# atomicarchitects/equiformer

Hardware: AMD Instinct MI355X
Metric: molecules/sec (train step) QM9 L_max=2, 6 blocks (higher is better)
Workload: dtype f32; 1 GPU; QM9 graph_attention_transformer_nonlinear_l2 train step (radius graph + fwd + L1 + bwd + AdamW), 128 molecules/GPU x 18 atoms, r=5.0, num_basis=128, alpha_drop=0.2; global_batch=128, nodes_per_gpu=2304, edges_per_gpu=25354, parallelism=dp1, matrix_mode=split, hip_graph=True, hip_graph_replays=449, hip_graph_eager_steps=3

## Files before the change

### equiformer_amd/csrc/edge.hip

```cpp
#include "common.h"
#include "prof.h"

namespace {

__global__ __launch_bounds__(256) void gather_add_kernel(const float* __restrict__ a, const float* __restrict__ b,
                                                         const int* __restrict__ src, const int* __restrict__ dst,
                                                         float* __restrict__ msg, long total4, int D4) {
  const long idx = (long)blockIdx.x * blockDim.x + threadIdx.x;
  if (idx >= total4) return;
  const long e = idx / D4;
  const int c = (int)(idx - e * D4);
  float4 v = reinterpret_cast<const float4*>(a)[(long)src[e] * D4 + c];
  if (b) {
    const float4 w = reinterpret_cast<const float4*>(b)[(long)dst[e] * D4 + c];
    v.x += w.x, v.y += w.y, v.z += w.z, v.w += w.w;
  }
  reinterpret_cast<float4*>(msg)[idx] = v;
}

__global__ __launch_bounds__(128) void segment_sum_kernel(const float* __restrict__ x, const int* __restrict__ ptr,
                                                          const int* __restrict__ perm, float* __restrict__ out, int D,
                                                          float scale, int accumulate) {
  const int n = blockIdx.x;
  const int beg = ptr[n], end = ptr[n + 1];
  if ((D & 3) == 0) {
    const int D4 = D >> 2;
    for (int c = threadIdx.x; c < D4; c += blockDim.x) {
      float4 acc = make_float4(0.f, 0.f, 0.f, 0.f);
      for (int q = beg; q < end; q += 4) {
        long row[4];
        float4 v[4];
#pragma unroll
        for (int j = 0; j < 4; ++j) {
          const int qq = min(q + j, end - 1);
          row[j] = perm ? perm[qq] : qq;
        }
#pragma unroll
        for (int j = 0; j < 4; ++j) v[j] = reinterpret_cast<const float4*>(x)[row[j] * D4 + c];
#pragma unroll
        for (int j = 0; j < 4; ++j)
          if (q + j < end) acc.x += v[j].x, acc.y += v[j].y, acc.z += v[j].z, acc.w += v[j].w;
      }
      acc.x *= scale, acc.y *= scale, acc.z *= scale, acc.w *= scale;
      float4* o = reinterpret_cast<float4*>(out) + (long)n * D4 + c;
      if (accumulate) {
        const float4 p = *o;
        acc.x += p.x, acc.y += p.y, acc.z += p.z, acc.w += p.w;
      }
      *o = acc;
    }
  } else {
    for (int c = threadIdx.x; c < D; c += blockDim.x) {
      float acc = 0.f;
      for (int q = beg; q < end; ++q) {
        const long row = perm ? perm[q] : q;
        acc += x[row * D + c];
      }
      acc *= scale;
      float* o = out + (long)n * D + c;
      *o = accumulate ? *o + acc : acc;
    }
  }
}

__global__ __launch_bounds__(256) void segment_bcast_kernel(const float* __restrict__ x, const int* __restrict__ seg_of,
                                                            float* __restrict__ out, long total, int D, float scale) {
  const long idx = (long)blockIdx.x * blockDim.x + threadIdx.x;
  if (idx >= total) return;
  const long row = idx / D;
  const int c = (int)(idx - row * D);
  out[idx] = scale * x[(long)seg_of[row] * D + c];
}

__global__ __launch_bounds__(256) void segment_scale_kernel(const float* __restrict__ x, const float* __restrict__ s,
                                                            const int* __restrict__ seg_of, float* __restrict__ out,
                                                            long total4, int D4) {
  const long idx = (long)blockIdx.x * blockDim.x + threadIdx.x;
  if (idx >= total4) return;
  const long row = idx / D4;
  const float f = s[seg_of[row]];
  float4 v = reinterpret_cast<const float4*>(x)[idx];
  v.x *= f; v.y *= f; v.z *= f; v.w *= f;
  reinterpret_cast<float4*>(out)[idx] = v;
}

// ... 454 lines not shown

int eqf_gather_add_fwd(const float* a, const float* b, const int* src, const int* dst, float* msg, int E, int D,
                       void* stream) {
  if (!a || !src || !msg || (b && !dst)) return EQF_E_BADARG;
  if (D % 4 != 0) return EQF_E_UNSUPPORTED;
  if (E <= 0) return 0;
  const long total4 = (long)E * (D / 4);
  hipLaunchKernelGGL(gather_add_kernel, dim3(eqf_cdiv(total4, 256)), dim3(256), 0, (hipStream_t)stream, a, b, src, dst,
                     msg, total4, D / 4);
  EQF_CHECK_LAUNCH();
  return 0;
}

int eqf_segment_sum(const float* x, const int* ptr, const int* perm, float* out, int nseg, int D, float scale,
                    int accumulate, void* stream) {
  if (!x || !ptr || !out) return EQF_E_BADARG;
  if (nseg <= 0 || D <= 0) return 0;
  hipLaunchKernelGGL(segment_sum_kernel, dim3(nseg), dim3(128), 0, (hipStream_t)stream, x, ptr, perm, out, D, scale,
                     accumulate);
  EQF_CHECK_LAUNCH();
  return 0;
}

int eqf_segment_scale(const float* x, const float* s, const int* seg_of, float* out, int rows, int D, void* stream) {
  if (!x || !s || !seg_of || !out) return EQF_E_BADARG;
  if (D % 4) return EQF_E_UNSUPPORTED;
  if (rows <= 0 || D <= 0) return 0;
  const long total4 = (long)rows * (D / 4);
  hipLaunchKernelGGL(segment_scale_kernel, dim3(eqf_cdiv(total4, 256)), dim3(256), 0, (hipStream_t)stream, x, s, seg_of,
                     out, total4, D / 4);
  EQF_CHECK_LAUNCH();
  return 0;
}

int eqf_segment_bcast(const float* x, const int* seg_of, float* out, int rows, int D, float scale, void* stream) {
  if (!x || !seg_of || !out) return EQF_E_BADARG;
  if (rows <= 0 || D <= 0) return 0;
  const long total = (long)rows * D;
  hipLaunchKernelGGL(segment_bcast_kernel, dim3(eqf_cdiv(total, 256)), dim3(256), 0, (hipStream_t)stream, x, seg_of,
                     out, total, D, scale);
  EQF_CHECK_LAUNCH();
  return 0;
}

int eqf_dtp_coupling_fwd(const float* sh, const float* cg, const eqf_dtp_paths* paths, float* coupling, int E,
                         void* stream) {
// ... 148 lines not shown
```

### equiformer_amd/csrc/rowops.hip

```cpp
#include "common.h"

namespace {

constexpr int WAVES_PER_BLOCK = 4;

struct SegTab {
  int nseg;
  int off[EQF_MAX_SEG];
  int len[EQF_MAX_SEG];
  int mul[EQF_MAX_SEG];
  int l[EQF_MAX_SEG];
  int woff[EQF_MAX_SEG];
  int boff[EQF_MAX_SEG];
  int zidx[EQF_MAX_SEG];
  int n0;
  int D;
};

SegTab make_segtab(const eqf_irreps& ir) {
  SegTab t{};
  t.nseg = ir.nseg;
  int off = 0, w = 0, b = 0, n0 = 0;
  for (int s = 0; s < ir.nseg; ++s) {
    t.off[s] = off;
// ... 79 lines not shown
      for (int i = lane; i < n; i += 64) sum += xs[i];
      mean = wave_sum(sum) / n;
    }
    float sg = 0.f, sgx = 0.f;
    for (int i = lane; i < n; i += 64) {
      const float g = gs[i] * ws[i % mul];
      const float xh = (xs[i] - mean) * rs;
      sg += g;
      sgx += g * xh;
    }
    sgx = wave_sum(sgx) / n;
    sg = (T.l[s] == 0) ? wave_sum(sg) / n : 0.f;
    for (int i = lane; i < n; i += 64) {
      const float g = gs[i] * ws[i % mul];
      const float xh = (xs[i] - mean) * rs;
      float v = rs * (g - sg - xh * sgx);
      if (rr) v += rr[T.off[s] + i];
      dr[T.off[s] + i] = v;
    }
  }
}

constexpr int LN_WGRAD_ROWS = 64, LN_WGRAD_CHUNK = 16;
__global__ __launch_bounds__(256) void layernorm_wgrad_kernel(const float* __restrict__ x, const float* __restrict__ dy,
                                                              const float* __restrict__ rstd,
                                                              const float* __restrict__ mean0, float* __restrict__ dw,
                                                              float* __restrict__ db, int rows, SegTab T) {
  constexpr int CH = LN_WGRAD_CHUNK;
  const int c = blockIdx.x * blockDim.x + threadIdx.x;
  if (c >= T.D) return;
  int s = 0;
  while (s + 1 < T.nseg && c >= T.off[s + 1]) ++s;
  const int u = (c - T.off[s]) % T.mul[s];
  const bool is0 = T.l[s] == 0;
  const int n0 = T.n0, z = T.zidx[s];
  float aw = 0.f, ab = 0.f;
  for (int r0 = blockIdx.y * LN_WGRAD_ROWS; r0 < min(rows, (int)(blockIdx.y + 1) * LN_WGRAD_ROWS); r0 += CH) {
    float gv[CH], xs[CH], rs[CH], m0[CH];
#pragma unroll
    for (int k = 0; k < CH; ++k) {
      const int r = min(r0 + k, rows - 1);
      gv[k] = dy[(long)r * T.D + c];
      xs[k] = x[(long)r * T.D + c];
      rs[k] = rstd[(long)r * T.nseg + s];
      m0[k] = is0 ? mean0[(long)r * n0 + z] : 0.f;
    }
#pragma unroll
    for (int k = 0; k < CH; ++k) {
      const float g = (r0 + k < rows) ? gv[k] : 0.f;
      aw += g * (xs[k] - m0[k]) * rs[k];
      ab += g;
    }
  }
  atomicAdd(dw + T.woff[s] + u, aw);
  if (T.boff[s] >= 0) atomicAdd(db + T.boff[s] + u, ab);
}

struct GateTab {
  int S, G, nseg;
  int in_off[EQF_MAX_SEG], out_off[EQF_MAX_SEG], goff[EQF_MAX_SEG], mul[EQF_MAX_SEG], d[EQF_MAX_SEG];
  int Din, Dout;
};

GateTab make_gatetab(int S, const eqf_irreps& gated) {
  GateTab t{};
  t.S = S;
  t.nseg = gated.nseg;
  int G = 0;
  for (int s = 0; s < gated.nseg; ++s) G += gated.mul[s];
  t.G = G;
  int in_off = S + G, out_off = S, g = 0;
  for (int s = 0; s < gated.nseg; ++s) {
    t.in_off[s] = in_off, t.out_off[s] = out_off, t.goff[s] = S + g;
    t.mul[s] = gated.mul[s], t.d[s] = 2 * gated.l[s] + 1;
    in_off += t.mul[s] * t.d[s], out_off += t.mul[s] * t.d[s], g += t.mul[s];
  }
  t.Din = in_off, t.Dout = out_off;
  return t;
// ... 443 lines not shown
int eqf_layernorm_fwd(const float* x, const float* weight, const float* bias, float* y, float* rstd, float* mean0,
                      int rows, const eqf_irreps* irreps, float eps, void* stream) {
  return eqf_add_layernorm_fwd(x, nullptr, nullptr, weight, bias, y, rstd, mean0, rows, irreps, eps, stream);
}

int eqf_add_layernorm_bwd(const float* x, const float* weight, const float* dy, const float* dres, const float* rstd,
                          const float* mean0, float* dx, float* d_weight, float* d_bias, int rows,
                          const eqf_irreps* irreps, void* stream) {
  if (!x || !weight || !dy || !rstd || !mean0 || !dx || !irreps || irreps->nseg < 1 || irreps->nseg > EQF_MAX_SEG)
    return EQF_E_BADARG;
  if (rows <= 0) return 0;
  const SegTab T = make_segtab(*irreps);
  hipLaunchKernelGGL(layernorm_bwd_kernel, dim3(eqf_cdiv(rows, WAVES_PER_BLOCK)), dim3(256), 0, (hipStream_t)stream, x,
                     weight, dy, dres, rstd, dx, rows, T);
  EQF_CHECK_LAUNCH();
  if (d_weight && d_bias) {
    hipLaunchKernelGGL(layernorm_wgrad_kernel, dim3(eqf_cdiv(T.D, 256), eqf_cdiv(rows, LN_WGRAD_ROWS)), dim3(256), 0,
                       (hipStream_t)stream, x, dy, rstd, mean0, d_weight, d_bias, rows, T);
    EQF_CHECK_LAUNCH();
  }
  return 0;
}

int eqf_layernorm_bwd(const float* x, const float* weight, const float* dy, const float* rstd, const float* mean0,
                      float* dx, float* d_weight, float* d_bias, int rows, const eqf_irreps* irreps, void* stream) {
  return eqf_add_layernorm_bwd(x, weight, dy, nullptr, rstd, mean0, dx, d_weight, d_bias, rows, irreps, stream);
}

int eqf_gate_fwd(const float* in, float* out, int rows, int S, const eqf_irreps* gated, float c_silu, float c_sig,
                 void* stream) {
  if (!in || !out || !gated) return EQF_E_BADARG;
  if (rows <= 0) return 0;
  const GateTab T = make_gatetab(S, *gated);
  const int RB = 8;
  hipLaunchKernelGGL(gate_fwd_cols_kernel, dim3(eqf_cdiv(rows, RB), eqf_cdiv(T.Dout, 256)), dim3(256), 0,
                     (hipStream_t)stream, in, out, rows, T, c_silu, c_sig, RB);
  EQF_CHECK_LAUNCH();
  return 0;
}

int eqf_gate_bwd(const float* in, const float* d_out, float* d_in, int rows, int S, const eqf_irreps* gated,
                 float c_silu, float c_sig, void* stream) {
  if (!in || !d_out || !d_in || !gated) return EQF_E_BADARG;
  for (int s = 0; s < gated->nseg; ++s)
    if (gated->l[s] > 3) return EQF_E_UNSUPPORTED;
  if (rows <= 0) return 0;
// ... 124 lines not shown
```

### equiformer_amd/lib.py

```python
import ctypes
import os

_HERE = os.path.dirname(os.path.abspath(__file__))
LIB_PATH = os.path.join(_HERE, "libequiformer_hip.so")
if os.environ.get("EQF_LIB_VARIANT"):
    LIB_PATH = os.path.join(_HERE, "libequiformer_hip_%s.so" % os.environ["EQF_LIB_VARIANT"])

EQF_MAX_SEG = 8
EQF_MAX_PATHS = 72
EQF_L3_ODD = 0x100

c_fp = ctypes.c_void_p
c_int = ctypes.c_int


class EqfIrreps(ctypes.Structure):
    _fields_ = [("nseg", c_int), ("l", c_int * EQF_MAX_SEG), ("mul", c_int * EQF_MAX_SEG), ("odd", c_int * EQF_MAX_SEG)]


class EqfRows(ctypes.Structure):
    _fields_ = [("d", c_int), ("ld", c_int), ("inner", c_int)]


class EqfGemmDesc(ctypes.Structure):
    _fields_ = [("A", c_fp), ("B", c_fp), ("C", c_fp), ("bias", c_fp), ("ra", EqfRows), ("rc", EqfRows),
                ("ldb", c_int), ("M", c_int), ("N", c_int), ("K", c_int), ("accumulate", c_int), ("kind", c_int)]


class EqfGateIn(ctypes.Structure):
    _fields_ = [("S", c_int), ("G", c_int), ("c_silu", ctypes.c_float), ("c_sig", ctypes.c_float)]


_PA = c_int * EQF_MAX_PATHS


class EqfDtpPaths(ctypes.Structure):
    _fields_ = [("npaths", c_int), ("sh_dim", c_int), ("in_dim", c_int), ("out_dim", c_int), ("w_numel", c_int),
                ("m_numel", c_int), ("l1", _PA), ("l2", _PA), ("l3", _PA), ("mul", _PA), ("in_off", _PA),
                ("out_off", _PA), ("out_ch", _PA), ("out_k", _PA), ("w_off", _PA), ("cg_off", _PA), ("m_off", _PA)]


_SA = c_int * EQF_MAX_SEG


class EqfEdgeDeg(ctypes.Structure):
    _fields_ = [("nblk", c_int), ("C", c_int), ("H", c_int), ("w_numel", c_int), ("pw_numel", c_int), ("m_numel", c_int),
                ("Z", c_int), ("D", c_int), ("l", _SA), ("N", _SA), ("K", _SA), ("w_off", _SA), ("out_ch", _SA),
                ("pw_off", _SA), ("m_off", _SA), ("node_off", _SA), ("z_off", _SA)]

# ... 38 lines not shown
    "eqf_dtp_coupling_fwd": [c_fp, c_fp, _P_PATHS, c_fp, c_int, c_fp],
    "eqf_dtp_coupling_bwd": [c_fp, c_fp, _P_PATHS, c_fp, c_int, c_fp],
    "eqf_dtp_linear_fwd": [c_fp, c_fp, c_fp, _P_PATHS, _PP, c_fp, c_fp, _P_IRR, c_int, c_fp],
    "eqf_dtp_linear_wgrad": [c_fp, c_fp, c_fp, _P_PATHS, c_fp, _P_IRR, _PP, c_int, c_fp],
    "eqf_sfc_fwd": [c_fp, c_fp, c_fp, _P_PATHS, _PP, c_fp, c_fp, c_fp, c_fp, _P_IRR, c_fp, c_int, c_int, c_fp],
    "eqf_sfc_bwd_data": [c_fp, c_fp, c_fp, _P_PATHS, _PP, c_fp, c_fp, _P_IRR, c_fp, c_int, c_fp, c_fp, c_fp, c_int, c_fp],
    "eqf_sfc_bwd_weight": [c_fp, c_fp, c_fp, _P_PATHS, c_fp, _P_IRR, c_fp, c_int, _PP, c_fp, c_int, c_fp],
    "eqf_sfcx_packed_numel": [_P_PATHS, _P_IRR, c_int, c_int],
    "eqf_sfcx_supported": [_P_PATHS, _P_IRR, c_int, c_int],
    "eqf_sfcx_fwd_gated": [c_fp, ctypes.POINTER(EqfGateIn), c_fp, c_fp, _P_PATHS, c_fp, c_fp, c_fp, _P_IRR, c_int, c_int, c_fp],
    "eqf_sfcx_bwd_data_gated": [c_fp, ctypes.POINTER(EqfGateIn), c_fp, c_fp, _P_PATHS, c_fp, c_fp, _P_IRR, c_fp, c_fp, c_fp,
                                c_int, c_int, c_fp],
    "eqf_sfcx_bwd_weight_gated": [c_fp, ctypes.POINTER(EqfGateIn), c_fp, c_fp, _P_PATHS, c_fp, _P_IRR, _PP, c_int, c_int,
                                  c_fp],
    "eqf_sfcx_bwd_weight_bias": [c_fp, c_fp, c_fp, _P_PATHS, c_fp, _P_IRR, c_fp, c_int, _PP, c_fp, c_fp, c_fp, c_int, c_int, c_fp],
    "eqf_sfcx_bwd_weight_gated_bias": [c_fp, ctypes.POINTER(EqfGateIn), c_fp, c_fp, _P_PATHS, c_fp, _P_IRR, _PP, c_fp, c_int,
                                       c_int, c_fp],
    "eqf_sfcx_pack": [_PP, c_fp, _P_PATHS, _P_IRR, c_int, c_int, c_fp, c_fp],
    "eqf_sfcx_fwd": [c_fp, c_fp, c_fp, _P_PATHS, c_fp, c_fp, c_fp, c_fp, _P_IRR, c_fp, c_int, c_int, c_int, c_fp],
    "eqf_sfcx_bwd_data": [c_fp, c_fp, c_fp, _P_PATHS, c_fp, c_fp, _P_IRR, c_fp, c_int, c_fp, c_fp, c_fp, c_int, c_int, c_fp],
    "eqf_sfcx_bwd_weight": [c_fp, c_fp, c_fp, _P_PATHS, c_fp, _P_IRR, c_fp, c_int, _PP, c_fp, c_int, c_int, c_fp],
    "eqf_layernorm_fwd": [c_fp, c_fp, c_fp, c_fp, c_fp, c_fp, c_int, _P_IRR, _f, c_fp],
    "eqf_layernorm_bwd": [c_fp, c_fp, c_fp, c_fp, c_fp, c_fp, c_fp, c_fp, c_int, _P_IRR, c_fp],
    "eqf_add_layernorm_fwd": [c_fp, c_fp, c_fp, c_fp, c_fp, c_fp, c_fp, c_fp, c_int, _P_IRR, _f, c_fp],
    "eqf_add_layernorm_bwd": [c_fp, c_fp, c_fp, c_fp, c_fp, c_fp, c_fp, c_fp, c_fp, c_int, _P_IRR, c_fp],
    "eqf_graphnorm_fwd": [c_fp, c_fp, c_fp, c_fp, c_fp, c_fp, c_fp, c_fp, c_fp, c_fp, c_fp, c_int, c_int, _P_IRR, _f, c_fp],
    "eqf_graphnorm_bwd": [c_fp, c_fp, c_fp, c_fp, c_fp, c_fp, c_fp, c_fp, c_fp, c_fp, c_fp, c_fp, c_fp, c_fp, c_int, c_int,
                          _P_IRR, c_fp],
    "eqf_gate_fwd": [c_fp, c_fp, c_int, c_int, _P_IRR, _f, _f, c_fp],
    "eqf_gate_bwd": [c_fp, c_fp, c_fp, c_int, c_int, _P_IRR, _f, _f, c_fp],
    "eqf_silu_fwd": [c_fp, c_fp, _long, _f, c_fp],
    "eqf_silu_bwd": [c_fp, c_fp, c_fp, _long, _f, c_fp],
    "eqf_lnsilu_fwd": [c_fp, c_fp, c_fp, c_fp, c_int, c_int, _f, c_fp],
    "eqf_lnsilu_bwd": [c_fp, c_fp, c_fp, c_fp, c_fp, c_fp, c_fp, c_int, c_int, _f, c_fp],
    "eqf_lnsilu_group_fwd": [c_fp, c_fp, c_fp, c_fp, c_int, c_int, c_int, _f, c_fp],
    "eqf_lnsilu_group_bwd": [c_fp, c_fp, c_fp, c_fp, c_fp, c_fp, c_fp, c_int, c_int, c_int, _f, c_fp],
    "eqf_fold_weight_fwd": [c_fp, c_fp, c_fp, c_fp, c_fp, c_int, c_fp],
    "eqf_fold_weight_bwd": [c_fp, c_fp, c_fp, c_fp, c_fp, c_fp, c_fp, c_int, c_fp],
    "eqf_embed_fwd": [c_fp, c_fp, c_fp, c_fp, c_int, c_int, c_int, c_fp],
    "eqf_embed_bwd": [c_fp, c_fp, c_fp, c_fp, c_int, c_int, c_int, c_fp],
    "eqf_gather_add_fwd": [c_fp, c_fp, c_fp, c_fp, c_fp, c_int, c_int, c_fp],
    "eqf_segment_sum": [c_fp, c_fp, c_fp, c_fp, c_int, c_int, _f, c_int, c_fp],
    "eqf_segment_bcast": [c_fp, c_fp, c_fp, c_int, c_int, _f, c_fp],
    "eqf_kv_split": [c_fp, c_fp, c_fp, c_int, c_int, c_fp, c_fp],
    "eqf_kv_merge": [c_fp, c_fp, c_fp, c_int, c_int, c_fp, c_fp],
    "eqf_dp_logits_fwd": [c_fp, c_fp, c_fp, c_fp, c_int, c_int, c_fp, c_fp],
    "eqf_dp_logits_bwd": [c_fp, c_fp, c_fp, c_fp, c_fp, c_fp, c_int, c_int, c_fp, c_fp],
    "eqf_vec_sh": [c_fp, c_fp, c_int, c_int, _f, c_fp, c_fp],
    "eqf_edgedeg_fold_fwd": [c_fp, c_fp, c_fp, c_fp, c_fp, _P_EDEG, c_fp, c_fp, c_fp],
    "eqf_edgedeg_fold_bwd": [c_fp, c_fp, c_fp, c_fp, c_fp, _P_EDEG, c_fp, c_fp, c_fp, c_fp, c_fp, c_fp, c_fp],
    "eqf_edgedeg_scatter_fwd": [c_fp, c_fp, c_fp, c_fp, _P_EDEG, _f, c_fp, c_int, c_int, c_fp],
    "eqf_edgedeg_scatter_bwd": [c_fp, c_fp, c_fp, c_fp, _P_EDEG, _f, c_fp, c_fp, c_int, c_int, c_fp],
    "eqf_segment_scale": [c_fp, c_fp, c_fp, c_fp, c_int, c_int, c_fp],
    "eqf_dtp_fwd": [c_fp, c_fp, c_fp, _P_PATHS, c_fp, c_int, c_fp],
    "eqf_dtp_bwd": [c_fp, c_fp, c_fp, _P_PATHS, c_fp, c_fp, c_fp, c_fp, c_int, c_fp],
    "eqf_alpha_fwd": [c_fp, c_fp, c_fp, c_int, c_int, c_int, _f, c_fp],
    "eqf_alpha_bwd": [c_fp, c_fp, c_fp, c_fp, c_fp, c_int, c_int, c_int, _f, c_fp],
    "eqf_attn_aggregate_fwd": [c_fp, c_fp, c_fp, c_fp, c_fp, c_int, c_int, _P_IRR, _f, _u64, c_fp],
    "eqf_attn_aggregate_bwd": [c_fp, c_fp, c_fp, c_fp, c_fp, c_fp, c_int, c_int, _P_IRR, _f, _u64, c_fp],
    "eqf_attn_aggregate_fwd_dseed": [c_fp, c_fp, c_fp, c_fp, c_fp, c_int, c_int, _P_IRR, _f, _u64, c_fp, c_fp],
    "eqf_attn_aggregate_bwd_dseed": [c_fp, c_fp, c_fp, c_fp, c_fp, c_fp, c_int, c_int, _P_IRR, _f, _u64, c_fp, c_fp],
    "eqf_silu_bwd2": [c_fp, c_fp, c_fp, c_fp, c_fp, _long, _f, c_fp],
    "eqf_gate_bwd2": [c_fp, c_fp, c_fp, c_fp, c_fp, c_int, c_int, _P_IRR, _f, _f, c_fp],
    "eqf_lnsilu_bwd2": [c_fp, c_fp, c_fp, c_fp, c_fp, c_fp, c_fp, c_fp, c_fp, c_int, c_int, _f, c_fp],
    "eqf_lnsilu_group_bwd2": [c_fp, c_fp, c_fp, c_fp, c_fp, c_fp, c_fp, c_fp, c_fp, c_int, c_int, c_int, _f, c_fp],
# ... 111 lines not shown
```

### equiformer_amd/ops.py

```python
import contextlib
import ctypes
import os
import weakref

import torch
from torch.autograd import Function
from torch.autograd.function import once_differentiable

from . import lib
from .lib import EqfGemmDesc, EqfRows, call


class HipOnlyError(RuntimeError):
    pass


_dummy = {}


class _Flag:
    on = False


_input_grads_only = _Flag()


class input_grads_only:

    def __enter__(self):
        self.prev = _input_grads_only.on
        _input_grads_only.on = True

    def __exit__(self, *exc):
# ... 163 lines not shown
        n = x.shape[0]
        y = torch.empty_like(x)
        rstd = torch.empty((n, len(layout.segs)), device=x.device, dtype=torch.float32)
        mean0 = torch.empty((n, _ln_means(layout)), device=x.device, dtype=torch.float32)
        call("eqf_layernorm_fwd", _p(x), _p(weight), _p(bias), _p(y), _p(rstd), _p(mean0), n, layout.c_ref,
             float(eps), _stream())
        ctx.save_for_backward(x, weight, rstd, mean0, bias)
        ctx.layout = layout
        ctx.nb = bias.numel()
        ctx.eps = eps
        return y

    @staticmethod
    def backward(ctx, dy):
        x, weight, rstd, mean0, bias = ctx.saved_tensors
        if torch.is_grad_enabled():
            dx, dw, db = _LayerNormBwd.apply(x, weight, dy, rstd, mean0, ctx.layout, ctx.eps, ctx.nb)
            return dx, _guard(dw, dy, "layer-norm weight gradient"), _guard(db, dy, "layer-norm bias gradient"), \
                None, None
        dy = _c(dy)
        _chk(dy)
        dx = torch.empty_like(x)
        dw, db = _zeros2(weight.numel(), ctx.nb, x.device)
        call("eqf_layernorm_bwd", _p(x), _p(weight), _p(dy), _p(rstd), _p(mean0), _p(dx), _p(dw), _p(db), x.shape[0],
             ctx.layout.c_ref, _stream())
        return dx, dw, db, None, None


class _LayerNormBwd(Function):

    @staticmethod
    def forward(ctx, x, weight, dy, rstd, mean0, layout, eps, nb):
        dy = _c(dy)
        _chk(dy)
        dx = torch.empty_like(x)
        want = _want_param_grads()
        dw, db = _zeros2(weight.numel(), nb, x.device) if want else (None, None)
        call("eqf_layernorm_bwd", _p(x), _p(weight), _p(dy), _p(rstd), _p(mean0), _p(dx), _p(dw), _p(db), x.shape[0],
             layout.c_ref, _stream())
        ctx.save_for_backward(x, weight, dy)
        ctx.layout, ctx.eps = layout, eps
        if not want:
            return dx, None, None
        ctx.mark_non_differentiable(dw, db)
        return dx, dw, db

    @staticmethod
    @once_differentiable
# ... 5 lines not shown
        g_w = _zeros_like(weight)
        call("eqf_layernorm_bwd2", _p(x), _p(weight), _p(dy), _p(c), _p(g_x), _p(g_w), _p(g_dy), x.shape[0],
             ctx.layout.c_ref, float(ctx.eps), _stream())
        return g_x, g_w, g_dy, None, None, None, None, None


def layer_norm(x, weight, bias, layout, eps=1e-5):
    return _LayerNorm.apply(x, weight, bias, layout, eps)


class _AddLayerNorm(Function):

    @staticmethod
    def forward(ctx, a, b, weight, bias, layout, eps):
        a, b = _c(a), _c(b)
        _chk(a, b, weight, bias)
        n = a.shape[0]
        s = torch.empty_like(a)
        y = torch.empty_like(a)
        rstd = torch.empty((n, len(layout.segs)), device=a.device, dtype=torch.float32)
        mean0 = torch.empty((n, _ln_means(layout)), device=a.device, dtype=torch.float32)
        call("eqf_add_layernorm_fwd", _p(a), _p(b), _p(s), _p(weight), _p(bias), _p(y), _p(rstd), _p(mean0), n,
             layout.c_ref, float(eps), _stream())
        ctx.save_for_backward(s, weight, rstd, mean0)
        ctx.layout, ctx.nb, ctx.eps = layout, bias.numel(), eps
        return s, y

    @staticmethod
    def backward(ctx, ds, dy):
        s, weight, rstd, mean0 = ctx.saved_tensors
        if dy is None:
            return ds, ds, None, None, None, None
        if torch.is_grad_enabled():
            dx, dw, db = _LayerNormBwd.apply(s, weight, dy, rstd, mean0, ctx.layout, ctx.eps, ctx.nb)
            d = dx if ds is None else dx + ds
            return d, d, _guard(dw, dy, "layer-norm weight gradient"), _guard(db, dy, "layer-norm bias gradient"), \
                None, None
        dy = _c(dy)
        ds = _c(ds) if ds is not None else None
        _chk(dy, ds)
        d = torch.empty_like(s)
        want = _want_param_grads()
        dw, db = _zeros2(weight.numel(), ctx.nb, s.device) if want else (None, None)
        call("eqf_add_layernorm_bwd", _p(s), _p(weight), _p(dy), _p(ds), _p(rstd), _p(mean0), _p(d), _p(dw), _p(db), s.shape[0],
             ctx.layout.c_ref, _stream())
        return d, d, dw, db, None, None


def add_layer_norm(a, b, weight, bias, layout, eps=1e-5):
    return _AddLayerNorm.apply(a, b, weight, bias, layout, eps)


def _gn_graph(graph, n):
    if graph is None or getattr(graph, "batch", None) is None or getattr(graph, "mol_ptr", None) is None:
        raise ValueError("the graph / instance norm needs the batch's EdgeGraph (graph=...) with batch and mol_ptr")
    if graph.batch.shape[0] != n or graph.num_graphs <= 0:
        raise ValueError("graph norm: %d rows, but the graph has %d nodes in %d graphs"
                         % (n, graph.batch.shape[0], graph.num_graphs))
    _chk(graph.mol_ptr, graph.batch)
    return graph.mol_ptr, graph.batch, int(graph.num_graphs)


def _gn_fwd(a, b, mean_shift, weight, bias, layout, graph, eps):
    _chk(a, b, mean_shift, weight, bias)
    n = a.shape[0]
    mol_ptr, batch, B = _gn_graph(graph, n)
    s = torch.empty_like(a) if b is not None else None
    y = torch.empty_like(a)
# ... 166 lines not shown
                           n * d, K, N))
    return dx, descs


def _lin_dgrad(dy, weight, spec):
    dx, descs = _lin_dgrad_descs(dy, weight, spec)
    _gemm_group(descs, _stream())
    return dx


def _lin_wgrad_descs(x, dy, spec, dw, db=None):
    n = x.shape[0]
    Din, Dout = spec.in_layout.dim, spec.out_layout.dim
    descs = []
    for (l, in_off, K, out_off, N, w_off) in spec.pairs:
        d = 2 * l + 1
        descs.append(_desc(2, (x, in_off), rows(d, Din, K), (dy, out_off), N, (dw, w_off), rows(d, Dout, N),
                           db if spec.has_bias(l, out_off) else None, K, N, n * d))
    return descs



_defer_wgrad = [os.environ.get("EQF_DEFER_WGRAD", "1") != "0"]
_defer_stats = {"queued": 0, "flushes": 0}


class _TaskQueue:
    __slots__ = ("entries", "__weakref__")

    def __init__(self):
        self.entries = []


_task_queues = weakref.WeakValueDictionary()


def set_deferred_weight_gradients(on):
    prev = _defer_wgrad[0]
    _defer_wgrad[0] = bool(on)
    return prev


def deferred_weight_gradient_stats(reset=False):
    out = dict(_defer_stats)
    if reset:
        _defer_stats["queued"] = _defer_stats["flushes"] = 0
    return out


def _alias(t):
    return (t.untyped_storage(), t.storage_offset(), t.numel(), t.device)


def _from_alias(a):
    stor, off, n, dev = a
    return torch.empty(0, dtype=torch.float32, device=dev).set_(stor, off, (n,))


def _launch_queue(q, early=False):
    entries, q.entries = q.entries, []
    if early:
        ready = [e for e in entries if e[0].grad is not None and (not e[5] or e[1].grad is not None)]
        q.entries = [e for e in entries if not (e[0].grad is not None and (not e[5] or e[1].grad is not None))]
        entries = ready
    descs = []
    for (w, b, x, dy, spec, fused_b, aw, ab) in entries:
        tw = _from_alias(aw)
        if w.grad is not None and w.grad.data_ptr() != tw.data_ptr():
            tw = w.grad.view(-1)
        tb = None
        if fused_b:
            tb = _from_alias(ab)
            if b.grad is not None and b.grad.data_ptr() != tb.data_ptr():
                tb = b.grad.view(-1)
        if not tw.is_contiguous() or tw.dtype != torch.float32 or (tb is not None and not tb.is_contiguous()):
            raise RuntimeError("deferred weight gradient: .grad must be a contiguous fp32 tensor")
        descs += _lin_wgrad_descs(x, dy, spec, tw, tb)
    if descs:
        _defer_stats["flushes"] += 1
        _gemm_group(descs, _stream())


def flush_deferred_weight_gradients():
    try:
        task = torch._C._current_graph_task_id()
    except Exception:
        return
    q = _task_queues.get(task)
    if q is not None and q.entries:
        _launch_queue(q, early=True)


def _hooked(p):
    if getattr(p, "_eqf_flushes", False):
        return False
    if getattr(p, "_backward_hooks", None) or getattr(p, "_post_accumulate_grad_hooks", None):
        return True
    dist = torch.distributed
    return bool(dist.is_available() and dist.is_initialized())


def _accumulates_into_grad(p):
    try:
        return bool(torch._C._will_engine_execute_node(torch.autograd.graph.get_gradient_edge(p).node))
    except RuntimeError:
        return False


def _can_defer(*params):
    return (_defer_wgrad[0] and not torch.is_grad_enabled()
            and all(p is None or (p.is_leaf and p.requires_grad and p.grad is None and not _hooked(p)
                                  and _accumulates_into_grad(p))
                    for p in params))


def _defer_lin_wgrad(w, b, x, dy, spec, fused_b, dw, db):
    task = torch._C._current_graph_task_id()
    q = _task_queues.get(task)
    if q is None:
        q = _TaskQueue()
        _task_queues[task] = q
        torch.autograd.Variable._execution_engine.queue_callback(lambda q=q: _launch_queue(q))
    q.entries.append((w, b, x, dy, spec, fused_b, _alias(dw), _alias(db) if fused_b else None))
    _defer_stats["queued"] += 1


def _launch(built):
    _gemm_group(built[1], _stream())
    return built[0]


def _lin_fwd(x, weight, bias, spec):
    return _launch(_lin_fwd_descs(x, weight, bias, spec))


def _lin_dgrad(dy, weight, spec):
    return _launch(_lin_dgrad_descs(dy, weight, spec))


def _lin_wgrad(x, dy, spec, dw, db=None):
    _gemm_group(_lin_wgrad_descs(x, dy, spec, dw, db), _stream())
    return dw


def _glin_fwd_descs(x, ldx, K, wide, Ws, bs, cols=None):
    G = len(Ws)
    cols = range(G) if cols is None else cols
# ... 718 lines not shown
        db = None
        if has_b and ctx.needs_input_grad[2] and _want_param_grads():
            db = torch.empty(spec.blocks[0]["N"], device=dnode.device, dtype=torch.float32)
        call("eqf_edgedeg_scatter_bwd", _p(dnode), _p(coupling), _p(graph.dst), _p(graph.row_ptr), spec.c_ref, scale, _p(dz),
             _p(db), graph.N, graph.E, _stream())
        return dz, None, db, None, None, None


def edgedeg_scatter(z, coupling, bias, graph, spec, scale):
    return _EdgeDegScatter.apply(z, coupling, bias, graph, spec, float(scale))


def _gather_add_fwd(a, b, graph):
    D = a.shape[1]
    msg = torch.empty((graph.E, D), device=a.device, dtype=torch.float32)
    call("eqf_gather_add_fwd", _p(a), _p(b), _p(graph.src), _p(graph.dst), _p(msg), graph.E, D, _stream())
    return msg


def _gather_add_bwd(dmsg, g, n, want_a, want_b):
    D = dmsg.shape[1]
    st = _stream()
    da = db = None
    if want_a:
        da = torch.empty((n, D), device=dmsg.device, dtype=torch.float32)
        call("eqf_segment_sum", _p(dmsg), _p(g.src_ptr), _p(g.src_perm), _p(da), n, D, 1.0, 0, st)
    if want_b:
        db = torch.empty((n, D), device=dmsg.device, dtype=torch.float32)
        call("eqf_segment_sum", _p(dmsg), _p(g.row_ptr), None, _p(db), n, D, 1.0, 0, st)
    return da, db


class _GatherAddBwd(Function):

    @staticmethod
    def forward(ctx, dmsg, graph, n, has_b):
        dmsg = _c(dmsg)
        _chk(dmsg)
        ctx.graph, ctx.has_b = graph, has_b
        da, db = _gather_add_bwd(dmsg, graph, n, True, has_b)
        if has_b:
            return da, db
        return da

    @staticmethod
    @once_differentiable
# ... 1384 lines not shown
```

### include/equiformer_hip.h

```cpp
#ifndef EQUIFORMER_HIP_H
#define EQUIFORMER_HIP_H

#ifdef __cplusplus
extern "C" {
#endif

#define EQF_MAX_SEG 8
#define EQF_MAX_PATHS 72

#define EQF_L3_ODD 0x100

#define EQF_E_BADARG (-1)
#define EQF_E_UNSUPPORTED (-2)

typedef struct eqf_irreps {
  int nseg;
  int l[EQF_MAX_SEG];
  int mul[EQF_MAX_SEG];
  int odd[EQF_MAX_SEG];
} eqf_irreps;

typedef struct eqf_dtp_paths {
  int npaths;
  int sh_dim;
// ... 129 lines not shown
                       const eqf_irreps* out1_irreps, int E, int mode, void* stream);
int eqf_sfcx_bwd_data_gated(const float* x_raw, const eqf_gate_in* gate, const float* coupling, const float* w,
                            const eqf_dtp_paths* paths, const void* packed, const float* d_out1,
                            const eqf_irreps* out1_irreps, float* d_x_raw, float* dw, float* d_coupling, int E, int mode,
                            void* stream);
int eqf_sfcx_bwd_weight_gated(const float* x_raw, const eqf_gate_in* gate, const float* coupling, const float* w,
                              const eqf_dtp_paths* paths, const float* d_out1, const eqf_irreps* out1_irreps,
                              float* const* dWl, int E, int mode, void* stream);

int eqf_sfcx_bwd_weight_bias(const float* x, const float* coupling, const float* w, const eqf_dtp_paths* paths,
                             const float* d_out1, const eqf_irreps* out1_irreps, const float* d_out2, int n2,
                             float* const* dWl, float* dW2, float* d_bias0, float* d_bias2, int E, int mode, void* stream);
int eqf_sfcx_bwd_weight_gated_bias(const float* x_raw, const eqf_gate_in* gate, const float* coupling, const float* w,
                                   const eqf_dtp_paths* paths, const float* d_out1, const eqf_irreps* out1_irreps,
                                   float* const* dWl, float* d_bias0, int E, int mode, void* stream);


int eqf_layernorm_fwd(const float* x, const float* weight, const float* bias, float* y, float* rstd,
                      float* mean0, int rows, const eqf_irreps* irreps, float eps, void* stream);
int eqf_layernorm_bwd(const float* x, const float* weight, const float* dy, const float* rstd,
                      const float* mean0, float* dx, float* d_weight, float* d_bias, int rows,
                      const eqf_irreps* irreps, void* stream);

int eqf_add_layernorm_fwd(const float* x, const float* x2, float* xsum, const float* weight, const float* bias,
                          float* y, float* rstd, float* mean0, int rows, const eqf_irreps* irreps, float eps,
                          void* stream);
int eqf_add_layernorm_bwd(const float* x, const float* weight, const float* dy, const float* dres, const float* rstd,
                          const float* mean0, float* dx, float* d_weight, float* d_bias, int rows,
                          const eqf_irreps* irreps, void* stream);

int eqf_graphnorm_fwd(const float* x, const float* x2, float* xsum, const float* mean_shift, const float* weight,
                      const float* bias, float* y, float* mean, float* rstd, const int* mol_ptr, const int* batch, int rows,
                      int num_graphs, const eqf_irreps* irreps, float eps, void* stream);
int eqf_graphnorm_bwd(const float* x, const float* mean_shift, const float* weight, const float* dy, const float* dres,
                      const float* mean, const float* rstd, const int* mol_ptr, const int* batch, float* dx,
                      float* d_weight, float* d_bias, float* d_mean_shift, double* workspace, int rows, int num_graphs,
                      const eqf_irreps* irreps, void* stream);

int eqf_gate_fwd(const float* in, float* out, int rows, int S, const eqf_irreps* gated, float c_silu,
                 float c_sig, void* stream);
int eqf_gate_bwd(const float* in, const float* d_out, float* d_in, int rows, int S,
                 const eqf_irreps* gated, float c_silu, float c_sig, void* stream);

int eqf_silu_fwd(const float* x, float* y, long n, float c, void* stream);
int eqf_silu_bwd(const float* x, const float* dy, float* dx, long n, float c, void* stream);

// ... 3 lines not shown
                   float* d_gamma, float* d_beta, int rows, int C, float eps, void* stream);

int eqf_lnsilu_group_fwd(const float* x, const float* gamma, const float* beta, float* y, int rows, int C, int groups,
                         float eps, void* stream);
int eqf_lnsilu_group_bwd(const float* x, const float* gamma, const float* beta, const float* dy, float* dx,
                         float* d_gamma, float* d_beta, int rows, int C, int groups, float eps, void* stream);

int eqf_fold_weight_fwd(const float* W, const float* w, const int* row_start, const int* w_of_row, float* out, int rows,
                        void* stream);
int eqf_fold_weight_bwd(const float* W, const float* w, const int* row_start, const int* w_of_row, const float* g,
                        float* dW, float* dw, int rows, void* stream);

int eqf_embed_fwd(const int* type, const float* W, const float* b, float* y, int rows, int C, int D,
                  void* stream);
int eqf_embed_bwd(const int* type, const float* dy, float* dW, float* db, int rows, int C, int D,
                  void* stream);


int eqf_gather_add_fwd(const float* a, const float* b, const int* src, const int* dst, float* msg,
                       int E, int D, void* stream);

int eqf_segment_sum(const float* x, const int* ptr, const int* perm, float* out, int nseg, int D,
                    float scale, int accumulate, void* stream);
int eqf_segment_bcast(const float* x, const int* seg_of, float* out, int rows, int D, float scale,
                      void* stream);

typedef struct eqf_edgedeg {
  int nblk;
  int C;
  int H;
  int w_numel;
  int pw_numel;
  int m_numel;
  int Z;
  int D;
  int l[EQF_MAX_SEG], N[EQF_MAX_SEG], K[EQF_MAX_SEG];
  int w_off[EQF_MAX_SEG], out_ch[EQF_MAX_SEG], pw_off[EQF_MAX_SEG], m_off[EQF_MAX_SEG], node_off[EQF_MAX_SEG];
  int z_off[EQF_MAX_SEG];
} eqf_edgedeg;
int eqf_edgedeg_fold_fwd(const float* W3, const float* offset, const float* exp_w, const float* exp_b, const float* W,
                         const eqf_edgedeg* desc, float* At, float* a, void* stream);
int eqf_edgedeg_fold_bwd(const float* W3, const float* offset, const float* exp_w, const float* exp_b, const float* W,
                         const eqf_edgedeg* desc, const float* dAt, const float* da, float* dW3, float* doffset, float* dW,
                         float* dx0, void* stream);
int eqf_edgedeg_scatter_fwd(const float* z, const float* coupling, const int* row_ptr, const float* bias,
                            const eqf_edgedeg* desc, float scale, float* node, int nnodes, int E, void* stream);
// ... 96 lines not shown
```

Before: 14980 molecules/s.

## Batch layernorm weight-grad kernels into grouped launch and pair segment sums

Layernorm backward passes null weight/bias grads to the bwd kernel and queues the wgrad work, which is flushed at the end of backward as one grouped kernel covering up to 32 norms with a table-driven block-to-problem map. Gather-add backward that needs both src and dst gradients now runs one paired segment-sum kernel instead of two launches. The aim is fewer small kernel launches and better GPU fill. The cost is a larger kernarg struct, extra Python bookkeeping, and reliance on the deferred queue flushing correctly.

Result: faster. 15310 molecules/s, median of 6 (+2.2%).

```diff
diff --git a/equiformer_amd/csrc/edge.hip b/equiformer_amd/csrc/edge.hip
--- a/equiformer_amd/csrc/edge.hip
+++ b/equiformer_amd/csrc/edge.hip
@@ -18,10 +18,9 @@
   reinterpret_cast<float4*>(msg)[idx] = v;
 }
 
-__global__ __launch_bounds__(128) void segment_sum_kernel(const float* __restrict__ x, const int* __restrict__ ptr,
-                                                          const int* __restrict__ perm, float* __restrict__ out, int D,
-                                                          float scale, int accumulate) {
-  const int n = blockIdx.x;
+__device__ __forceinline__ void segment_sum_block(const float* __restrict__ x, const int* __restrict__ ptr,
+                                                  const int* __restrict__ perm, float* __restrict__ out, int D,
+                                                  float scale, int accumulate, int n) {
   const int beg = ptr[n], end = ptr[n + 1];
   if ((D & 3) == 0) {
     const int D4 = D >> 2;
@@ -61,6 +60,22 @@
       *o = accumulate ? *o + acc : acc;
     }
   }
+}
+
+__global__ __launch_bounds__(128) void segment_sum_kernel(const float* __restrict__ x, const int* __restrict__ ptr,
+                                                          const int* __restrict__ perm, float* __restrict__ out, int D,
+                                                          float scale, int accumulate) {
+  segment_sum_block(x, ptr, perm, out, D, scale, accumulate, (int)blockIdx.x);
+}
+
+__global__ __launch_bounds__(128) void segment_sum_pair_kernel(const float* __restrict__ x, const int* __restrict__ ptr_a,
+                                                               const int* __restrict__ perm_a, float* __restrict__ out_a,
+                                                               const int* __restrict__ ptr_b,
+                                                               const int* __restrict__ perm_b, float* __restrict__ out_b,
+                                                               int nseg, int D) {
+  const int b = (int)blockIdx.x;
+  if (b < nseg) segment_sum_block(x, ptr_a, perm_a, out_a, D, 1.f, 0, b);
+  else segment_sum_block(x, ptr_b, perm_b, out_b, D, 1.f, 0, b - nseg);
 }
 
 __global__ __launch_bounds__(256) void segment_bcast_kernel(const float* __restrict__ x, const int* __restrict__ seg_of,
@@ -561,6 +576,16 @@
   return 0;
 }
 
+int eqf_segment_sum_pair(const float* x, const int* ptr_a, const int* perm_a, float* out_a, const int* ptr_b,
+                         const int* perm_b, float* out_b, int nseg, int D, void* stream) {
+  if (!x || !ptr_a || !out_a || !ptr_b || !out_b || out_a == out_b) return EQF_E_BADARG;
+  if (nseg <= 0 || D <= 0) return 0;
+  hipLaunchKernelGGL(segment_sum_pair_kernel, dim3(2 * nseg), dim3(128), 0, (hipStream_t)stream, x, ptr_a, perm_a, out_a,
+                     ptr_b, perm_b, out_b, nseg, D);
+  EQF_CHECK_LAUNCH();
+  return 0;
+}
+
 int eqf_segment_scale(const float* x, const float* s, const int* seg_of, float* out, int rows, int D, void* stream) {
   if (!x || !s || !seg_of || !out) return EQF_E_BADARG;
   if (D % 4) return EQF_E_UNSUPPORTED;
diff --git a/equiformer_amd/csrc/rowops.hip b/equiformer_amd/csrc/rowops.hip
--- a/equiformer_amd/csrc/rowops.hip
+++ b/equiformer_amd/csrc/rowops.hip
@@ -1,3 +1,5 @@
+#include <limits.h>
+#include <string.h>
 #include "common.h"
 
 namespace {
@@ -125,12 +127,12 @@
 }
 
 constexpr int LN_WGRAD_ROWS = 64, LN_WGRAD_CHUNK = 16;
-__global__ __launch_bounds__(256) void layernorm_wgrad_kernel(const float* __restrict__ x, const float* __restrict__ dy,
-                                                              const float* __restrict__ rstd,
-                                                              const float* __restrict__ mean0, float* __restrict__ dw,
-                                                              float* __restrict__ db, int rows, SegTab T) {
+__device__ __forceinline__ void layernorm_wgrad_block(const float* __restrict__ x, const float* __restrict__ dy,
+                                                      const float* __restrict__ rstd, const float* __restrict__ mean0,
+                                                      float* __restrict__ dw, float* __restrict__ db, int rows,
+                                                      const SegTab& T, int bx, int by) {
   constexpr int CH = LN_WGRAD_CHUNK;
-  const int c = blockIdx.x * blockDim.x + threadIdx.x;
+  const int c = bx * 256 + threadIdx.x;
   if (c >= T.D) return;
   int s = 0;
   while (s + 1 < T.nseg && c >= T.off[s + 1]) ++s;
@@ -138,7 +140,7 @@
   const bool is0 = T.l[s] == 0;
   const int n0 = T.n0, z = T.zidx[s];
   float aw = 0.f, ab = 0.f;
-  for (int r0 = blockIdx.y * LN_WGRAD_ROWS; r0 < min(rows, (int)(blockIdx.y + 1) * LN_WGRAD_ROWS); r0 += CH) {
+  for (int r0 = by * LN_WGRAD_ROWS; r0 < min(rows, (by + 1) * LN_WGRAD_ROWS); r0 += CH) {
     float gv[CH], xs[CH], rs[CH], m0[CH];
 #pragma unroll
     for (int k = 0; k < CH; ++k) {
@@ -157,6 +159,39 @@
   }
   atomicAdd(dw + T.woff[s] + u, aw);
   if (T.boff[s] >= 0) atomicAdd(db + T.boff[s] + u, ab);
+}
+
+__global__ __launch_bounds__(256) void layernorm_wgrad_kernel(const float* __restrict__ x, const float* __restrict__ dy,
+                                                              const float* __restrict__ rstd,
+                                                              const float* __restrict__ mean0, float* __restrict__ dw,
+                                                              float* __restrict__ db, int rows, SegTab T) {
+  layernorm_wgrad_block(x, dy, rstd, mean0, dw, db, rows, T, (int)blockIdx.x, (int)blockIdx.y);
+}
+
+constexpr int LNG_MAXP = 32, LNG_MAXT = 4;
+struct LNGP {
+  const float *x, *dy, *rstd, *mean0;
+  float *dw, *db;
+  int rows, tab;
+};
+struct LNGroup {
+  int n;
+  int woff[LNG_MAXP + 1];
+  SegTab tab[LNG_MAXT];
+  LNGP p[LNG_MAXP];
+};
+static_assert(sizeof(LNGroup) <= 4000, "kernarg segment");
+
+__global__ __launch_bounds__(256) void layernorm_wgrad_group_kernel(LNGroup g) {
+  const int b = (int)blockIdx.x;
+  int pi = 0;
+#pragma unroll
+  for (int j = 1; j < LNG_MAXP; ++j) pi += (int)((unsigned)(g.woff[j] - 1 - b) >> 31);
+  const LNGP& P = g.p[pi];
+  const SegTab& T = g.tab[P.tab];
+  const int local = b - g.woff[pi], nx = (T.D + 255) / 256;
+  const int by = local / nx;
+  layernorm_wgrad_block(P.x, P.dy, P.rstd, P.mean0, P.dw, P.db, P.rows, T, local - by * nx, by);
 }
 
 struct GateTab {
@@ -646,6 +681,42 @@
   return 0;
 }
 
+int eqf_layernorm_wgrad_group(const eqf_ln_wgrad_desc* d, int n, void* stream) {
+  if (n < 0 || (n > 0 && !d)) return EQF_E_BADARG;
+  for (int i = 0; i < n; ++i) {
+    if (d[i].rows <= 0) continue;
+    if (!d[i].x || !d[i].dy || !d[i].rstd || !d[i].mean0 || !d[i].d_weight || !d[i].d_bias || !d[i].irreps ||
+        d[i].irreps->nseg < 1 || d[i].irreps->nseg > EQF_MAX_SEG)
+      return EQF_E_BADARG;
+  }
+  static thread_local LNGroup G;
+  int i = 0;
+  while (i < n) {
+    memset(&G, 0, sizeof G);
+    int ntab = 0, wg = 0;
+    for (; i < n && G.n < LNG_MAXP; ++i) {
+      if (d[i].rows <= 0) continue;
+      const SegTab T = make_segtab(*d[i].irreps);
+      int t = 0;
+      while (t < ntab && memcmp(&G.tab[t], &T, sizeof T) != 0) ++t;
+      if (t == ntab) {
+        if (ntab == LNG_MAXT) break;
+        G.tab[ntab++] = T;
+      }
+      LNGP& P = G.p[G.n];
+      P.x = d[i].x, P.dy = d[i].dy, P.rstd = d[i].rstd, P.mean0 = d[i].mean0;
+      P.dw = d[i].d_weight, P.db = d[i].d_bias, P.rows = d[i].rows, P.tab = t;
+      G.woff[G.n++] = wg;
+      wg += eqf_cdiv(T.D, 256) * eqf_cdiv(d[i].rows, LN_WGRAD_ROWS);
+    }
+    if (!G.n) continue;
+    for (int j = G.n; j <= LNG_MAXP; ++j) G.woff[j] = j == G.n ? wg : INT_MAX;
+    hipLaunchKernelGGL(layernorm_wgrad_group_kernel, dim3(wg), dim3(256), 0, (hipStream_t)stream, G);
+    EQF_CHECK_LAUNCH();
+  }
+  return 0;
+}
+
 int eqf_layernorm_bwd(const float* x, const float* weight, const float* dy, const float* rstd, const float* mean0,
                       float* dx, float* d_weight, float* d_bias, int rows, const eqf_irreps* irreps, void* stream) {
   return eqf_add_layernorm_bwd(x, weight, dy, nullptr, rstd, mean0, dx, d_weight, d_bias, rows, irreps, stream);
diff --git a/equiformer_amd/lib.py b/equiformer_amd/lib.py
--- a/equiformer_amd/lib.py
+++ b/equiformer_amd/lib.py
@@ -25,6 +25,11 @@
 class EqfGemmDesc(ctypes.Structure):
     _fields_ = [("A", c_fp), ("B", c_fp), ("C", c_fp), ("bias", c_fp), ("ra", EqfRows), ("rc", EqfRows),
                 ("ldb", c_int), ("M", c_int), ("N", c_int), ("K", c_int), ("accumulate", c_int), ("kind", c_int)]
+
+
+class EqfLnWgradDesc(ctypes.Structure):
+    _fields_ = [("x", c_fp), ("dy", c_fp), ("rstd", c_fp), ("mean0", c_fp), ("d_weight", c_fp), ("d_bias", c_fp),
+                ("rows", c_int), ("irreps", ctypes.POINTER(EqfIrreps))]
 
 
 class EqfGateIn(ctypes.Structure):
@@ -109,6 +114,7 @@
     "eqf_sfcx_bwd_weight": [c_fp, c_fp, c_fp, _P_PATHS, c_fp, _P_IRR, c_fp, c_int, _PP, c_fp, c_int, c_int, c_fp],
     "eqf_layernorm_fwd": [c_fp, c_fp, c_fp, c_fp, c_fp, c_fp, c_int, _P_IRR, _f, c_fp],
     "eqf_layernorm_bwd": [c_fp, c_fp, c_fp, c_fp, c_fp, c_fp, c_fp, c_fp, c_int, _P_IRR, c_fp],
+    "eqf_layernorm_wgrad_group": [ctypes.POINTER(EqfLnWgradDesc), c_int, c_fp],
     "eqf_add_layernorm_fwd": [c_fp, c_fp, c_fp, c_fp, c_fp, c_fp, c_fp, c_fp, c_int, _P_IRR, _f, c_fp],
     "eqf_add_layernorm_bwd": [c_fp, c_fp, c_fp, c_fp, c_fp, c_fp, c_fp, c_fp, c_fp, c_int, _P_IRR, c_fp],
     "eqf_graphnorm_fwd": [c_fp, c_fp, c_fp, c_fp, c_fp, c_fp, c_fp, c_fp, c_fp, c_fp, c_fp, c_int, c_int, _P_IRR, _f, c_fp],
@@ -128,6 +134,7 @@
     "eqf_embed_bwd": [c_fp, c_fp, c_fp, c_fp, c_int, c_int, c_int, c_fp],
     "eqf_gather_add_fwd": [c_fp, c_fp, c_fp, c_fp, c_fp, c_int, c_int, c_fp],
     "eqf_segment_sum": [c_fp, c_fp, c_fp, c_fp, c_int, c_int, _f, c_int, c_fp],
+    "eqf_segment_sum_pair": [c_fp, c_fp, c_fp, c_fp, c_fp, c_fp, c_fp, c_int, c_int, c_fp],
     "eqf_segment_bcast": [c_fp, c_fp, c_fp, c_int, c_int, _f, c_fp],
     "eqf_kv_split": [c_fp, c_fp, c_fp, c_int, c_int, c_fp, c_fp],
     "eqf_kv_merge": [c_fp, c_fp, c_fp, c_int, c_int, c_fp, c_fp],
diff --git a/equiformer_amd/ops.py b/equiformer_amd/ops.py
--- a/equiformer_amd/ops.py
+++ b/equiformer_amd/ops.py
@@ -8,7 +8,7 @@
 from torch.autograd.function import once_differentiable
 
 from . import lib
-from .lib import EqfGemmDesc, EqfRows, call
+from .lib import EqfGemmDesc, EqfLnWgradDesc, EqfRows, call
 
 
 class HipOnlyError(RuntimeError):
@@ -218,8 +218,11 @@
         _chk(dy)
         dx = torch.empty_like(x)
         dw, db = _zeros2(weight.numel(), ctx.nb, x.device)
-        call("eqf_layernorm_bwd", _p(x), _p(weight), _p(dy), _p(rstd), _p(mean0), _p(dx), _p(dw), _p(db), x.shape[0],
-             ctx.layout.c_ref, _stream())
+        defer = _can_defer(weight, bias)
+        call("eqf_layernorm_bwd", _p(x), _p(weight), _p(dy), _p(rstd), _p(mean0), _p(dx), None if defer else _p(dw),
+             None if defer else _p(db), x.shape[0], ctx.layout.c_ref, _stream())
+        if defer:
+            _defer_norm_wgrad(weight, bias, x, dy, rstd, mean0, ctx.layout, dw, db)
         return dx, dw, db, None, None
 
 
@@ -271,13 +274,13 @@
         mean0 = torch.empty((n, _ln_means(layout)), device=a.device, dtype=torch.float32)
         call("eqf_add_layernorm_fwd", _p(a), _p(b), _p(s), _p(weight), _p(bias), _p(y), _p(rstd), _p(mean0), n,
              layout.c_ref, float(eps), _stream())
-        ctx.save_for_backward(s, weight, rstd, mean0)
+        ctx.save_for_backward(s, weight, rstd, mean0, bias)
         ctx.layout, ctx.nb, ctx.eps = layout, bias.numel(), eps
         return s, y
 
     @staticmethod
     def backward(ctx, ds, dy):
-        s, weight, rstd, mean0 = ctx.saved_tensors
+        s, weight, rstd, mean0, bias = ctx.saved_tensors
         if dy is None:
             return ds, ds, None, None, None, None
         if torch.is_grad_enabled():
@@ -291,8 +294,11 @@
         d = torch.empty_like(s)
         want = _want_param_grads()
         dw, db = _zeros2(weight.numel(), ctx.nb, s.device) if want else (None, None)
-        call("eqf_add_layernorm_bwd", _p(s), _p(weight), _p(dy), _p(ds), _p(rstd), _p(mean0), _p(d), _p(dw), _p(db), s.shape[0],
-             ctx.layout.c_ref, _stream())
+        defer = want and _can_defer(weight, bias)
+        call("eqf_add_layernorm_bwd", _p(s), _p(weight), _p(dy), _p(ds), _p(rstd), _p(mean0), _p(d),
+             None if defer else _p(dw), None if defer else _p(db), s.shape[0], ctx.layout.c_ref, _stream())
+        if defer:
+            _defer_norm_wgrad(weight, bias, s, dy, rstd, mean0, ctx.layout, dw, db)
         return d, d, dw, db, None, None
 
 
@@ -505,14 +511,15 @@
 
 
 _defer_wgrad = [os.environ.get("EQF_DEFER_WGRAD", "1") != "0"]
-_defer_stats = {"queued": 0, "flushes": 0}
+_defer_stats = {"queued": 0, "flushes": 0, "norms_queued": 0, "norm_flushes": 0}
 
 
 class _TaskQueue:
-    __slots__ = ("entries", "__weakref__")
+    __slots__ = ("entries", "norms", "__weakref__")
 
     def __init__(self):
         self.entries = []
+        self.norms = []
 
 
 _task_queues = weakref.WeakValueDictionary()
@@ -525,9 +532,10 @@
 
 
 def deferred_weight_gradient_stats(reset=False):
-    out = dict(_defer_stats)
+    out = {k: v for k, v in _defer_stats.items() if not k.startswith("norm") or _defer_stats["norms_queued"]}
     if reset:
-        _defer_stats["queued"] = _defer_stats["flushes"] = 0
+        for k in _defer_stats:
+            _defer_stats[k] = 0
     return out
 
 
@@ -562,6 +570,36 @@
     if descs:
         _defer_stats["flushes"] += 1
         _gemm_group(descs, _stream())
+    _launch_norm_queue(q, early)
+
+
+def _grad_target(p, a):
+    t = _from_alias(a)
+    if p.grad is not None and p.grad.data_ptr() != t.data_ptr():
+        t = p.grad.view(-1)
+    if not t.is_contiguous() or t.dtype != torch.float32:
+        raise RuntimeError("deferred weight gradient: .grad must be a contiguous fp32 tensor")
+    return t
+
+
+def _ln_wgrad_group(descs, st):
+    arr = (EqfLnWgradDesc * len(descs))()
+    for d, (x, dy, rstd, mean0, layout, dw, db) in zip(arr, descs):
+        d.x, d.dy, d.rstd, d.mean0, d.d_weight, d.d_bias = _p(x), _p(dy), _p(rstd), _p(mean0), _p(dw), _p(db)
+        d.rows, d.irreps = x.shape[0], ctypes.pointer(layout.c)
+    call("eqf_layernorm_wgrad_group", arr, len(descs), st)
+
+
+def _launch_norm_queue(q, early):
+    entries, q.norms = q.norms, []
+    if early:
+        q.norms = [e for e in entries if e[0].grad is None or e[1].grad is None]
+        entries = [e for e in entries if e[0].grad is not None and e[1].grad is not None]
+    descs = [(x, dy, rstd, mean0, layout, _grad_target(w, aw), _grad_target(b, ab))
+             for (w, b, x, dy, rstd, mean0, layout, aw, ab) in entries]
+    if descs:
+        _defer_stats["norm_flushes"] += 1
+        _ln_wgrad_group(descs, _stream())
 
 
 def flush_deferred_weight_gradients():
@@ -570,7 +608,7 @@
     except Exception:
         return
     q = _task_queues.get(task)
-    if q is not None and q.entries:
+    if q is not None and (q.entries or q.norms):
         _launch_queue(q, early=True)
 
 
@@ -597,15 +635,24 @@
                     for p in params))
 
 
-def _defer_lin_wgrad(w, b, x, dy, spec, fused_b, dw, db):
+def _task_queue():
     task = torch._C._current_graph_task_id()
     q = _task_queues.get(task)
     if q is None:
         q = _TaskQueue()
         _task_queues[task] = q
         torch.autograd.Variable._execution_engine.queue_callback(lambda q=q: _launch_queue(q))
-    q.entries.append((w, b, x, dy, spec, fused_b, _alias(dw), _alias(db) if fused_b else None))
+    return q
+
+
+def _defer_lin_wgrad(w, b, x, dy, spec, fused_b, dw, db):
+    _task_queue().entries.append((w, b, x, dy, spec, fused_b, _alias(dw), _alias(db) if fused_b else None))
     _defer_stats["queued"] += 1
+
+
+def _defer_norm_wgrad(weight, bias, x, dy, rstd, mean0, layout, dw, db):
+    _task_queue().norms.append((weight, bias, x, dy, rstd, mean0, layout, _alias(dw), _alias(db)))
+    _defer_stats["norms_queued"] += 1
 
 
 def _launch(built):
@@ -1370,6 +1417,11 @@
     D = dmsg.shape[1]
     st = _stream()
     da = db = None
+    if want_a and want_b:
+        da = torch.empty((n, D), device=dmsg.device, dtype=torch.float32)
+        db = torch.empty((n, D), device=dmsg.device, dtype=torch.float32)
+        call("eqf_segment_sum_pair", _p(dmsg), _p(g.src_ptr), _p(g.src_perm), _p(da), _p(g.row_ptr), None, _p(db), n, D, st)
+        return da, db
     if want_a:
         da = torch.empty((n, D), device=dmsg.device, dtype=torch.float32)
         call("eqf_segment_sum", _p(dmsg), _p(g.src_ptr), _p(g.src_perm), _p(da), n, D, 1.0, 0, st)
diff --git a/include/equiformer_hip.h b/include/equiformer_hip.h
--- a/include/equiformer_hip.h
+++ b/include/equiformer_hip.h
@@ -175,6 +175,14 @@
                       const float* mean0, float* dx, float* d_weight, float* d_bias, int rows,
                       const eqf_irreps* irreps, void* stream);
 
+typedef struct eqf_ln_wgrad_desc {
+  const float *x, *dy, *rstd, *mean0;
+  float *d_weight, *d_bias;
+  int rows;
+  const eqf_irreps* irreps;
+} eqf_ln_wgrad_desc;
+int eqf_layernorm_wgrad_group(const eqf_ln_wgrad_desc* descs, int n, void* stream);
+
 int eqf_add_layernorm_fwd(const float* x, const float* x2, float* xsum, const float* weight, const float* bias,
                           float* y, float* rstd, float* mean0, int rows, const eqf_irreps* irreps, float eps,
                           void* stream);
@@ -224,6 +232,8 @@
 
 int eqf_segment_sum(const float* x, const int* ptr, const int* perm, float* out, int nseg, int D,
                     float scale, int accumulate, void* stream);
+int eqf_segment_sum_pair(const float* x, const int* ptr_a, const int* perm_a, float* out_a, const int* ptr_b,
+                         const int* perm_b, float* out_b, int nseg, int D, void* stream);
 int eqf_segment_bcast(const float* x, const int* seg_of, float* out, int rows, int D, float scale,
                       void* stream);
 
```
